# esw0116/DynaVSR

Hardware: AMD Instinct MI355X
Metric: inner-loop frames/sec/GPU (EDVR-M x4, 5x3x180x320): forward leg = BASELINE.json configs[1]; the inner MAML step and the per-frame pipeline are `inner_step` / `per_frame_pipeline` (higher is better)
Workload: dtype f32; 1 GPU; EDVR-M x4 forward (PCD deformable alignment + TSA fusion + reconstruction), clips of 1x5x3x180x320 -> 3x720x1280 (BASELINE.json configs[1]); one step = 2 clip(s) per GPU, one per HIP stream (adapt.super_resolve_video); clips_in_flight_per_gpu=2

## Files before the change

### dynavsr_amd/csrc/conv2d_wino5.hip

```cpp
#include <type_traits>

#include "common.h"
#include "kernels.h"
#include "small_grid.h"

namespace dvsr {

#ifdef DVSR_CONV_TRACE
#define W5_STAMP(i)                                                                                       \
  do {                                                                                                    \
    if (a.trace && threadIdx.x == 0) a.trace[(size_t)blockIdx.x * 64 + (i)] = __builtin_readcyclecounter(); \
  } while (0)
#else
#define W5_STAMP(i) \
  do {              \
  } while (0)
#endif

typedef float w5f2 __attribute__((ext_vector_type(2)));
typedef __bf16 w5bf8 __attribute__((ext_vector_type(8)));
typedef __bf16 w5bf2 __attribute__((ext_vector_type(2)));
typedef unsigned w5u4 __attribute__((ext_vector_type(4)));

constexpr int W5_PCH = 18 * 2 * 3 * 256;

template <int TC>
struct Wino5Shape {
  static constexpr int CC = 8, NTILE = 32, TRW = NTILE / TC, NT = 768;
  static constexpr int OH = 4 * TRW, OW = 4 * TC;
  static constexpr int IH = OH + 2, RP = OW + 8, GR = RP / 4;
  static constexpr int NG = CC * IH * GR;
  static constexpr int NI = (NG + NT - 1) / NT;
  static constexpr int RAWPAD = NI * NT * 4;
  static constexpr int VIMG = 36 * 3 * 32 * 4;
  static constexpr int XCH = 6 * 16 * 64 * 4;
  static constexpr int LOOP = 2 * RAWPAD + 2 * VIMG;
  static constexpr size_t LDS_BYTES = (size_t)(LOOP > XCH ? LOOP : XCH) * sizeof(float);
};

constexpr int w5_waitcnt(int vm, int lgkm) { return (vm & 15) | (7 << 4) | ((lgkm & 15) << 8) | ((vm >> 4) << 14); }

__device__ __forceinline__ unsigned w5_cvt_pk(float a, float b) {
  return __builtin_bit_cast(unsigned, __builtin_convertvector(w5f2{a, b}, w5bf2));
}
__device__ __forceinline__ void w5_dma16(__amdgpu_buffer_rsrc_t rs, float* lds, unsigned voff, unsigned soff) {
  __builtin_amdgcn_raw_ptr_buffer_load_lds(rs, (__attribute__((address_space(3))) void*)lds, 16, voff, soff, 0, 0);
}
__device__ __forceinline__ __amdgpu_buffer_rsrc_t w5_rsrc(const float* base, int num_records) {
  return __builtin_amdgcn_make_buffer_rsrc(const_cast<float*>(base), 0, num_records, 0x00020000);
}

__global__ void pack_weights_wino5_kernel(PackTable t) {
  const PackEntry& e = t.e[blockIdx.y];
  if (e.layout != PackLayout::WINO_F4) return;
  __bf16* const P16 = reinterpret_cast<__bf16*>(e.P);
  const size_t total = (size_t)e.ncb * e.nchunks * 512;
  constexpr double G[6][3] = {{1.0 / 4, 0, 0},          {-1.0 / 6, -1.0 / 6, -1.0 / 6}, {-1.0 / 6, 1.0 / 6, -1.0 / 6},
                              {1.0 / 24, 1.0 / 12, 1.0 / 6}, {1.0 / 24, -1.0 / 12, 1.0 / 6}, {0, 0, 1}};
  for (size_t i = blockIdx.x * (size_t)blockDim.x + threadIdx.x; i < total; i += (size_t)gridDim.x * blockDim.x) {
    const int c8 = (int)(i & 7), col = (int)((i >> 3) & 63);
    const size_t ck = i >> 9;
    const int k = (int)(ck % e.nchunks), cb = (int)(ck / e.nchunks);
    const int co = cb * 64 + col, ci = k * 8 + c8;
    double g[3][3];
    const bool ok = co < e.Cout && ci < e.Ctot;
    const float* src = !e.wt ? e.w + ((size_t)co * (e.w_ctot ? e.w_ctot : e.Ctot) + (e.w_ctot ? e.w_coff : 0) + ci) * 9
                             : e.w + ((size_t)ci * e.w_ctot + e.w_coff + co) * 9;
#pragma unroll
    for (int tap = 0; tap < 9; ++tap) g[tap / 3][tap % 3] = ok ? (double)src[e.wt ? 8 - tap : tap] : 0.0;
    double c[6][3];
#pragma unroll
    for (int xi = 0; xi < 6; ++xi)
#pragma unroll
      for (int b = 0; b < 3; ++b) c[xi][b] = G[xi][0] * g[0][b] + G[xi][1] * g[1][b] + G[xi][2] * g[2][b];
    const int mh = col >> 5, c32 = col & 31;
    __bf16* dst = P16 + ck * (size_t)(2 * W5_PCH) + (size_t)mh * 1536 + (size_t)c32 * 8 + c8;
#pragma unroll
    for (int xi = 0; xi < 6; ++xi)
#pragma unroll
      for (int nu = 0; nu < 6; ++nu) {
        const float u = (float)(c[xi][0] * G[nu][0] + c[xi][1] * G[nu][1] + c[xi][2] * G[nu][2]);
        const __bf16 h = (__bf16)u;
        const float r1 = u - (float)h;
        const __bf16 m = (__bf16)r1;
        const __bf16 l = (__bf16)(r1 - (float)m);
        __bf16* d = dst + (size_t)(xi * 3 + (nu >> 1)) * 3072;
        if (nu & 1) { d[512] = m; d[768] = h; d[1024] = l; }
        else { d[0] = h; d[256] = m; d[1280] = l; }
      }
  }
}

int pack_weights_wino5_run(const PackTable& t, hipStream_t st) {
  hipLaunchKernelGGL(pack_weights_wino5_kernel, dim3(64, t.n), dim3(256), 0, st, t);
  return check_launch("pack_weights_wino5_kernel");
}

template <int TC, bool RES, bool R16, bool PRE>
__global__ __launch_bounds__(1024) void conv2d_wino5_kernel(ConvK2 a) {
  static_assert(!PRE || (R16 && !RES), "the addend is read by the sixteen-reader epilogue, never beside a residual");
  using Sh = Wino5Shape<TC>;
  constexpr int IH = Sh::IH, RP = Sh::RP, GR = Sh::GR;
  constexpr int CHF = IH * RP;
  constexpr int QF = 768 * 4;
  extern __shared__ __attribute__((aligned(16))) float smem[];
  float* const raw0 = smem;
  unsigned* const vimg0 = reinterpret_cast<unsigned*>(smem + 2 * Sh::RAWPAD);

  const int id = blockIdx.x;
  const int q_ = id >> 3;
  const int cbi = q_ % a.ncb;
  const int j_ = q_ / a.ncb;
  const int tile = (id & 7) * a.tiles_per_xcd + j_;
  if (j_ >= a.tiles_per_xcd || tile >= a.ntiles) return;
  const int tx_ = tile % a.tiles_x;
  const int t2 = tile / a.tiles_x;
  const int ty_ = t2 % a.tiles_y;
  const int n = t2 / a.tiles_y;
  const int oy0 = ty_ * Sh::OH, ox0 = tx_ * Sh::OW;

  const int tid = threadIdx.x, lane = tid & 63;
  const int wave = __builtin_amdgcn_readfirstlane(tid >> 6);
  const int lo = lane & 31, hi = lane >> 5;
  const size_t HW = (size_t)a.H * a.W;
  auto fence = [&]() __attribute__((always_inline)) { __builtin_amdgcn_sched_barrier(0); };
  auto lds_barrier = [&]() __attribute__((always_inline)) {
    asm volatile("s_waitcnt lgkmcnt(0)" ::: "memory");
    __builtin_amdgcn_s_barrier();
    asm volatile("" ::: "memory");
  };
  W5_STAMP(0);
#ifdef DVSR_CONV_TRACE
  if (a.trace && threadIdx.x == 0) a.trace[(size_t)blockIdx.x * 64 + 60] = __builtin_amdgcn_s_memrealtime();
#endif

  auto read16 = [&](int m) __attribute__((always_inline)) {
    int le = lane;
    asm volatile("" : "+v"(le));
    const int rq_r = wave & 3, cp_r = wave >> 2;
    const float* const xr = smem + (rq_r * 64 + le) * 4 + cp_r;
    const int lo_e = le & 31, hi_e = le >> 5;
    const int trow_e = lo_e / TC, tcol_e = lo_e - trow_e * TC;
    const int oy = oy0 + 4 * trow_e, ox = ox0 + 4 * tcol_e;
    const size_t HWo = (size_t)a.Ho * a.Wo;
    const float slope = a.act == ACT_LRELU ? 0.1f : (a.act == ACT_RELU ? 0.f : 1.f);
    const float* bias = wset_ptr(a.bias, a.b_gs, n, a.wdiv);
    const int co0 = cbi * 64 + m * 32 + 8 * rq_r + 4 * hi_e + cp_r;
    f32x4 pr[4];
    if constexpr (PRE) {
      const bool live = oy < a.Ho && ox < a.Wo && co0 < a.Cout;
      const float* pre = a.pre + (size_t)(n / a.pre_bdiv) * a.pre_bs + (size_t)co0 * HWo + (size_t)oy * a.Wo + ox;
#pragma unroll
      for (int i = 0; i < 4; ++i)
        pr[i] = (live && oy + i < a.Ho) ? *reinterpret_cast<const f32x4*>(pre + (size_t)i * a.Wo) : f32x4{0.f, 0.f, 0.f, 0.f};
    }
    float y[4][4];
#pragma unroll
    for (int j = 0; j < 4; ++j) {
      float z[6];
#pragma unroll
      for (int x = 0; x < 6; ++x) z[x] = xr[(x * 16 + j * 4) * 256];
      const float sa = z[1] + z[2], da = z[1] - z[2];
      const float sb = z[3] + z[4], db = z[3] - z[4];
      y[0][j] = z[0] + sa + sb;
      y[1][j] = __builtin_fmaf(2.f, db, da);
      y[2][j] = __builtin_fmaf(4.f, sb, sa);
      y[3][j] = __builtin_fmaf(8.f, db, da) + z[5];
    }
    const bool px_ok = oy < a.Ho && ox < a.Wo;
    const int nrow = a.Ho - oy < 4 ? a.Ho - oy : 4;
    if (px_ok && co0 < a.Cout) {
      const float b0 = bias ? bias[co0] : 0.f;
      const size_t base = ((size_t)n * a.Cout + co0) * HWo + (size_t)oy * a.Wo + ox;
      f32x4 rr[4];
      if constexpr (RES) {
#pragma unroll
        for (int i = 0; i < 4; ++i)
          rr[i] = i < nrow ? *reinterpret_cast<const f32x4*>(a.res + base + (size_t)i * a.Wo) : f32x4{0.f, 0.f, 0.f, 0.f};
      }
#pragma unroll
      for (int i = 0; i < 4; ++i) {
        if (i >= nrow) break;
        f32x4 v;
#pragma unroll
        for (int j = 0; j < 4; ++j) {
          float v0 = y[i][j] + b0;
          if constexpr (PRE) v0 += pr[i][j];
          v[j] = fmaxf(v0, v0 * slope);
        }
        if constexpr (RES) v += rr[i];
        *reinterpret_cast<f32x4*>(a.y + base + (size_t)i * a.Wo) = v;
      }
    }
  };

  if (wave >= 12) {
    const int pw = wave - 12, ptid = tid - 768;
    const float* x0n = a.x0 + (size_t)n * a.x0_bs;
    const float* x1n = a.c1 ? a.x1 + (size_t)(n / a.x1_bdiv) * a.x1_bs : x0n;
    static_assert(IH * GR * 4 == 720, "a channel quad is 720 groups");
    unsigned hoff[3];
#pragma unroll
    for (int jj = 0; jj < 3; ++jj) {
      const int L = jj * 256 + ptid;
      const int cq = L / (IH * GR), rr = L - cq * (IH * GR);
      const int iy = rr / GR, g = rr - iy * GR;
      const int gy = oy0 - 1 + iy, gx = ox0 - 4 + 4 * g;
      const bool live = L < 4 * IH * GR;
      const bool ok = live && (unsigned)gy < (unsigned)a.H && (unsigned)gx < (unsigned)a.W;
      hoff[jj] = ok ? (unsigned)(((size_t)cq * HW + (size_t)gy * a.W + gx) * 4) : 0x80000000u;
      if (live && !ok) {
#pragma unroll
        for (int bb = 0; bb < 4; ++bb) *reinterpret_cast<f32x4*>(raw0 + (bb >> 1) * Sh::RAWPAD + (bb & 1) * QF + L * 4) = f32x4{0.f, 0.f, 0.f, 0.f};
      }
    }
    const unsigned chunk_bytes = (unsigned)(Sh::CC * HW * 4), quad_bytes = (unsigned)(4 * HW * 4);
    auto issue_raw = [&](int k) __attribute__((always_inline)) {
      const bool live = k < a.nchunks;
      const bool second = k * Sh::CC >= a.c0;
      const unsigned soff = live ? (unsigned)(second ? k - a.c0 / Sh::CC : k) * chunk_bytes : 0u;
      const __amdgpu_buffer_rsrc_t rs = w5_rsrc(second ? x1n : x0n, live ? 0x7fffffff : 0);
      float* dst = raw0 + (k & 1) * Sh::RAWPAD + 256 * pw;
#pragma unroll
      for (int jj = 0; jj < 3; ++jj) {
        w5_dma16(rs, dst + jj * 1024, hoff[jj], soff);
        w5_dma16(rs, dst + QF + jj * 1024, hoff[jj], soff + quad_bytes);
      }
    };
    const int ptile = 8 * pw + (lane & 7), ppair = (lane >> 3) & 3;
    const int trow_t = ptile / TC, tcol_t = ptile - trow_t * TC;
    const int pch = 2 * ppair + hi;
    const float* prd = raw0 + (pch >> 2) * QF + (pch & 3) * CHF + 4 * trow_t * RP + 4 * tcol_t;
    unsigned* vw12 = vimg0 + (hi ? 2 : 1) * 6 * 384 + ptile * 4 + ppair;
    unsigned* vw34 = vimg0 + (hi ? 4 : 3) * 6 * 384 + ptile * 4 + ppair;
    unsigned* vw05 = vimg0 + (hi ? 5 : 0) * 6 * 384 + ptile * 4 + ppair;
    auto ld_row = [&](float (&d)[6], int row) __attribute__((always_inline)) {
      const float* p = prd + row * RP;
      const w5f2 l2 = *reinterpret_cast<const w5f2*>(p + 2);
      const f32x4 m4 = *reinterpret_cast<const f32x4*>(p + 4);
      const w5f2 h2 = *reinterpret_cast<const w5f2*>(p + 8);
      d[0] = l2[1]; d[1] = m4[0]; d[2] = m4[1]; d[3] = m4[2]; d[4] = m4[3]; d[5] = h2[0];
    };
    auto colpass = [&](const float (&r)[6], float (&v)[6]) __attribute__((always_inline)) {
      v[0] = __builtin_fmaf(4.f, r[0], __builtin_fmaf(-5.f, r[2], r[4]));
      v[5] = __builtin_fmaf(4.f, r[1], __builtin_fmaf(-5.f, r[3], r[5]));
      const float e1 = __builtin_fmaf(-4.f, r[2], r[4]), o1 = __builtin_fmaf(-4.f, r[1], r[3]);
      v[1] = e1 + o1; v[2] = e1 - o1;
      const float e2 = r[4] - r[2], o2 = r[3] - r[1];
      v[3] = __builtin_fmaf(2.f, o2, e2); v[4] = __builtin_fmaf(-2.f, o2, e2);
    };
    auto finish_pair = [&](const float (&ra)[6], const float (&rb)[6], unsigned* vw) __attribute__((always_inline)) {
      float va[6], vb[6];
      colpass(ra, va);
      colpass(rb, vb);
#pragma unroll
      for (int v = 0; v < 6; ++v) {
        const auto s0 = __builtin_amdgcn_permlane32_swap(__builtin_bit_cast(unsigned, va[v]), __builtin_bit_cast(unsigned, vb[v]), false, false);
        const unsigned u0 = s0[0], u1 = s0[1];
        const float v0 = __builtin_bit_cast(float, u0), v1 = __builtin_bit_cast(float, u1);
        const unsigned h = w5_cvt_pk(v0, v1);
        const float r0 = v0 - __builtin_bit_cast(float, h << 16), r1 = v1 - __builtin_bit_cast(float, h & 0xffff0000u);
        const unsigned m = w5_cvt_pk(r0, r1);
        const float q0 = r0 - __builtin_bit_cast(float, m << 16), q1 = r1 - __builtin_bit_cast(float, m & 0xffff0000u);
        unsigned* d = vw + v * 384;
#ifdef W5_NOVW
        d[0] = h ^ m ^ w5_cvt_pk(q0, q1);
#else
        d[0] = h; d[128] = m; d[256] = w5_cvt_pk(q0, q1);
#endif
      }
    };
    auto produce = [&]() __attribute__((always_inline)) {
      float d0[6], d1[6], d2[6], d3[6], d4[6], d5[6];
      ld_row(d1, 1); ld_row(d2, 2); ld_row(d3, 3); ld_row(d4, 4);
      ld_row(d0, 0); ld_row(d5, 5);
      float ra[6], rb[6];
#pragma unroll
      for (int j = 0; j < 6; ++j) {
        const float e = __builtin_fmaf(-4.f, d2[j], d4[j]), o = __builtin_fmaf(-4.f, d1[j], d3[j]);
        ra[j] = e + o; rb[j] = e - o;
      }
      finish_pair(ra, rb, vw12);
      fence();
#pragma unroll
      for (int j = 0; j < 6; ++j) {
        const float e = d4[j] - d2[j], o = d3[j] - d1[j];
        ra[j] = __builtin_fmaf(2.f, o, e); rb[j] = __builtin_fmaf(-2.f, o, e);
      }
      finish_pair(ra, rb, vw34);
      fence();
#pragma unroll
      for (int j = 0; j < 6; ++j) {
        ra[j] = __builtin_fmaf(4.f, d0[j], __builtin_fmaf(-5.f, d2[j], d4[j]));
        rb[j] = __builtin_fmaf(4.f, d1[j], __builtin_fmaf(-5.f, d3[j], d5[j]));
      }
      finish_pair(ra, rb, vw05);
    };
    issue_raw(0);
    issue_raw(1);
    __builtin_amdgcn_s_waitcnt(w5_waitcnt(6, 0));
    __builtin_amdgcn_s_barrier();
    asm volatile("" ::: "memory");
    produce();
    __builtin_amdgcn_s_waitcnt(w5_waitcnt(0, 0));
    __builtin_amdgcn_s_barrier();
    asm volatile("" ::: "memory");
    int vstep = Sh::VIMG, rstep = Sh::RAWPAD;
    vw12 += vstep; vw34 += vstep; vw05 += vstep; prd += rstep;
    __builtin_amdgcn_s_setprio(3);
    for (int k = 0; k < a.nchunks; ++k) {

#ifndef W5_NODMA
      issue_raw(k + 2);
#endif
#ifndef W5_NOPROD
      if (k + 1 < a.nchunks) produce();
#endif
      __builtin_amdgcn_s_waitcnt(w5_waitcnt(0, 0));
      __builtin_amdgcn_s_barrier();
      asm volatile("" ::: "memory");
      vw12 -= vstep; vw34 -= vstep; vw05 -= vstep; prd -= rstep;
      vstep = -vstep; rstep = -rstep;
    }
    if constexpr (R16) {
      __builtin_amdgcn_s_setprio(0);
      lds_barrier();
      lds_barrier(); read16(0);
      lds_barrier();
      lds_barrier(); read16(1);
    } else {
      lds_barrier(); lds_barrier(); lds_barrier(); lds_barrier();
    }
    return;
  }
  {
    const int cxi = wave % 6, cmh = wave / 6;
    f32x16 acc[6];
#pragma unroll
    for (int v = 0; v < 6; ++v)
#pragma unroll
      for (int r = 0; r < 16; ++r) acc[v][r] = 0.f;
    const float* wp_cb = wset_ptr(a.wp, a.w_gs, n, a.wdiv) + (size_t)cbi * a.nchunks * W5_PCH;
    const __amdgpu_buffer_rsrc_t wrsrc = w5_rsrc(wp_cb, -1);
    const unsigned avoff = (unsigned)(lane * 16);
    const int asb = (cxi * 3 * 2 + cmh) * 3072;
    f32x4 AF[3];
    auto gldA = [&](auto g_, int k) __attribute__((always_inline)) {
      constexpr int G = decltype(g_)::value;
#ifdef W5_NOA
      if (k > 0 || G > 2) return;
#endif
      const int soff = k * (W5_PCH * 4) + asb + (G / 3) * 6144 + (G % 3) * 1024;
      AF[G % 3] = __builtin_bit_cast(f32x4, __builtin_amdgcn_raw_buffer_load_b128(wrsrc, (int)avoff, soff, 0));
    };
    auto blend = [&](f32x4& x, const f32x4& l, bool keep) __attribute__((always_inline)) {
#pragma unroll
      for (int r = 0; r < 4; ++r) x[r] = keep ? x[r] : l[r];
    };
    const unsigned* vrd = vimg0 + cxi * 6 * 384 + lo * 4;
    const unsigned* vrd_lh = vrd + (hi ? 0 : 256);
    const unsigned* vrd_hl = vrd + (hi ? 256 : 0);
    w5u4 BF[2];
    auto ldB = [&](auto f_) __attribute__((always_inline)) {
      constexpr int F = decltype(f_)::value, NU = F / 3, W = F % 3;
      if constexpr (W == 0) BF[F & 1] = *reinterpret_cast<const w5u4*>(vrd + NU * 384);
      else if constexpr (W == 1) BF[F & 1] = *reinterpret_cast<const w5u4*>(vrd + NU * 384 + 128);
      else if constexpr (NU & 1) BF[F & 1] = *reinterpret_cast<const w5u4*>(vrd_hl + NU * 384);
      else BF[F & 1] = *reinterpret_cast<const w5u4*>(vrd_lh + NU * 384);
    };
    auto mma = [&](f32x16& c, const f32x4& av, const w5u4& bv) __attribute__((always_inline)) {
#ifdef W5_NOMMA
      c[0] += av[0] * __builtin_bit_cast(float, bv[0]);
      return;
#endif
      c = __builtin_amdgcn_mfma_f32_32x32x16_bf16(__builtin_bit_cast(w5bf8, av), __builtin_bit_cast(w5bf8, bv), c, 0, 0, 0);
    };
    static_for<0, 3>([&](auto g_) __attribute__((always_inline)) { gldA(g_, 0); });
    __builtin_amdgcn_s_barrier();
    asm volatile("" ::: "memory");
    __builtin_amdgcn_s_barrier();
    asm volatile("" ::: "memory");
    int vstep = Sh::VIMG;
    for (int k = 0; k < a.nchunks; ++k) {
      ldB(std::integral_constant<int, 0>{}); ldB(std::integral_constant<int, 1>{});
      const int knext = k + 1 < a.nchunks ? k + 1 : k;
      static_for<0, 18>([&](auto f_) __attribute__((always_inline)) {
        constexpr int F = decltype(f_)::value, NU = F / 3, I = F % 3;
        constexpr int XS = NU & 1;
        mma(acc[NU], AF[XS], BF[F & 1]);
#ifdef W5_NOBR
        if constexpr (false)
#else
        if constexpr (F + 2 < 18)
#endif
          ldB(std::integral_constant<int, (F + 2 < 18 ? F + 2 : 0)>{});
        if constexpr (I == 1) {
          blend(AF[XS], AF[2], (NU & 1) ? hi != 0 : hi == 0);
          if constexpr ((NU & 1) && NU < 5) gldA(std::integral_constant<int, 3 * ((NU < 5 ? NU : 1) / 2) + 5>{}, k);
          if constexpr (NU == 5) gldA(std::integral_constant<int, 2>{}, knext);
        }
        if constexpr (I == 2) {
          if constexpr (NU < 4) gldA(std::integral_constant<int, 3 * ((NU < 4 ? NU : 0) / 2) + 3 + (NU & 1)>{}, k);
          else gldA(std::integral_constant<int, (NU & 1)>{}, knext);
        }
        fence();
      });
      lds_barrier();
      if (k < 16) W5_STAMP(3 + k);
      vrd += vstep; vrd_lh += vstep; vrd_hl += vstep;
      vstep = -vstep;
    }
  W5_STAMP(40);

  int lane_e = lane;
  asm volatile("" : "+v"(lane_e));
  f32x16 Z[4];
#pragma unroll
  for (int r = 0; r < 16; ++r) {
    const float sa = acc[1][r] + acc[2][r], da = acc[1][r] - acc[2][r];
    const float sb = acc[3][r] + acc[4][r], db = acc[3][r] - acc[4][r];
    Z[0][r] = acc[0][r] + sa + sb;
    Z[1][r] = __builtin_fmaf(2.f, db, da);
    Z[2][r] = __builtin_fmaf(4.f, sb, sa);
    Z[3][r] = __builtin_fmaf(8.f, db, da) + acc[5][r];
  }
  float* const xw = smem + (cxi * 16 * 64 + lane_e) * 4;
  const int rq_r = wave & 3, cp_r = wave >> 2;
  const float* const xr = smem + (rq_r * 64 + lane_e) * 4 + cp_r * 2;
  const int lo_e = lane_e & 31, hi_e = lane_e >> 5;
  const int trow_e = lo_e / TC, tcol_e = lo_e - trow_e * TC;
  const int oy = oy0 + 4 * trow_e, ox = ox0 + 4 * tcol_e;
  const size_t HWo = (size_t)a.Ho * a.Wo;
  const float slope = a.act == ACT_LRELU ? 0.1f : (a.act == ACT_RELU ? 0.f : 1.f);
  const float* bias = wset_ptr(a.bias, a.b_gs, n, a.wdiv);
  W5_STAMP(50);
  lds_barrier();
  W5_STAMP(51);
#pragma unroll 1
  for (int m = 0; m < 2; ++m) {
    if (cmh == m) {
#pragma unroll
      for (int j = 0; j < 4; ++j)
#pragma unroll
        for (int rq = 0; rq < 4; ++rq)
          *reinterpret_cast<f32x4*>(xw + (j * 4 + rq) * 256) = f32x4{Z[j][4 * rq], Z[j][4 * rq + 1], Z[j][4 * rq + 2], Z[j][4 * rq + 3]};
    }
    W5_STAMP(52 + 4 * m);
    lds_barrier();
    W5_STAMP(53 + 4 * m);
    if constexpr (R16) read16(m);
    else if (wave < 8) {
      const int co0 = cbi * 64 + m * 32 + 8 * rq_r + 4 * hi_e + 2 * cp_r;
      float y[2][4][4];
#pragma unroll
      for (int j = 0; j < 4; ++j) {
        w5f2 z[6];
#pragma unroll
        for (int x = 0; x < 6; ++x) z[x] = *reinterpret_cast<const w5f2*>(xr + (x * 16 + j * 4) * 256);
#pragma unroll
        for (int c = 0; c < 2; ++c) {
          const float sa = z[1][c] + z[2][c], da = z[1][c] - z[2][c];
          const float sb = z[3][c] + z[4][c], db = z[3][c] - z[4][c];
          y[c][0][j] = z[0][c] + sa + sb;
          y[c][1][j] = __builtin_fmaf(2.f, db, da);
          y[c][2][j] = __builtin_fmaf(4.f, sb, sa);
          y[c][3][j] = __builtin_fmaf(8.f, db, da) + z[5][c];
        }
      }
      const bool px_ok = oy < a.Ho && ox < a.Wo;
      const int nrow = a.Ho - oy < 4 ? a.Ho - oy : 4;
      if (px_ok && co0 < a.Cout) {
        const bool two = co0 + 1 < a.Cout;
        const float b0 = bias ? bias[co0] : 0.f, b1 = (bias && two) ? bias[co0 + 1] : 0.f;
#pragma unroll
        for (int i = 0; i < 4; ++i)
#pragma unroll
          for (int j = 0; j < 4; ++j) {
            const float v0 = y[0][i][j] + b0, v1 = y[1][i][j] + b1;
            y[0][i][j] = fmaxf(v0, v0 * slope);
            y[1][i][j] = fmaxf(v1, v1 * slope);
          }
        if (a.ps == 0) {
#pragma unroll
          for (int c = 0; c < 2; ++c) {
            if (c == 1 && !two) break;
            const size_t base = ((size_t)n * a.Cout + co0 + c) * HWo + (size_t)oy * a.Wo + ox;
            if constexpr (RES) {
              f32x4 rr[4];
#pragma unroll
              for (int i = 0; i < 4; ++i)
                rr[i] = i < nrow ? *reinterpret_cast<const f32x4*>(a.res + base + (size_t)i * a.Wo) : f32x4{0.f, 0.f, 0.f, 0.f};
#pragma unroll
              for (int i = 0; i < 4; ++i) {
                if (i >= nrow) break;
                const f32x4 v = f32x4{y[c][i][0], y[c][i][1], y[c][i][2], y[c][i][3]} + rr[i];
                *reinterpret_cast<f32x4*>(a.y + base + (size_t)i * a.Wo) = v;
              }
            } else {
#pragma unroll
              for (int i = 0; i < 4; ++i) {
                if (i >= nrow) break;
                *reinterpret_cast<f32x4*>(a.y + base + (size_t)i * a.Wo) = f32x4{y[c][i][0], y[c][i][1], y[c][i][2], y[c][i][3]};
              }
            }
          }
        } else {
          const int cq = co0 >> 2, dy = (co0 >> 1) & 1;
          float* dst = a.y + (((size_t)n * (a.Cout >> 2) + cq) * (2 * a.Ho) + (2 * oy + dy)) * (size_t)(2 * a.Wo) + 2 * ox;
#pragma unroll
          for (int i = 0; i < 4; ++i) {
            if (i >= nrow) break;
            float* d = dst + (size_t)(2 * i) * (2 * a.Wo);
            *reinterpret_cast<f32x4*>(d) = f32x4{y[0][i][0], y[1][i][0], y[0][i][1], y[1][i][1]};
            *reinterpret_cast<f32x4*>(d + 4) = f32x4{y[0][i][2], y[1][i][2], y[0][i][3], y[1][i][3]};
          }
        }
      }
    }
    W5_STAMP(54 + 4 * m);
    if (m == 0) lds_barrier();
    W5_STAMP(55 + 4 * m);
  }
#ifdef DVSR_CONV_TRACE
  W5_STAMP(41);
  __builtin_amdgcn_s_waitcnt(0);
  W5_STAMP(42);
  if (a.trace && threadIdx.x == 0) {
    a.trace[(size_t)blockIdx.x * 64 + 61] = __builtin_amdgcn_s_memrealtime();
    a.trace[(size_t)blockIdx.x * 64 + 63] = __builtin_amdgcn_s_getreg((4) | (0 << 6) | (31 << 11));
    a.trace[(size_t)blockIdx.x * 64 + 62] = __builtin_amdgcn_s_getreg((20) | (0 << 6) | (31 << 11));
  }
#endif
  }
}

template <int TC>
static int launch_wino5(ConvK2 k, hipStream_t st) {
  using Sh = Wino5Shape<TC>;
  auto kern = k.pre ? conv2d_wino5_kernel<TC, false, true, true>
                    : (k.res ? conv2d_wino5_kernel<TC, true, true, false> : conv2d_wino5_kernel<TC, false, false, false>);
  static PerDeviceOnce attr_once, attr_once_r, attr_once_p;
  set_dyn_lds_once(attr_once, (const void*)conv2d_wino5_kernel<TC, false, false, false>, Sh::LDS_BYTES);
  set_dyn_lds_once(attr_once_r, (const void*)conv2d_wino5_kernel<TC, true, true, false>, Sh::LDS_BYTES);
  set_dyn_lds_once(attr_once_p, (const void*)conv2d_wino5_kernel<TC, false, true, true>, Sh::LDS_BYTES);
  k.tiles_x = ceil_div(k.Wo, Sh::OW); k.tiles_y = ceil_div(k.Ho, Sh::OH); k.ntiles = k.tiles_x * k.tiles_y * k.N;
  k.ncb = ceil_div(k.Cout, 64);
  k.tiles_per_xcd = ceil_div(k.ntiles, 8);
  k.nitems = k.tiles_per_xcd * 8 * k.ncb;
  hipLaunchKernelGGL(kern, dim3(k.nitems), dim3(1024), Sh::LDS_BYTES, st, k);
  return check_launch("conv2d_wino5_kernel");
}

int conv2d_wino5_launch(const ConvK2& k, int th, hipStream_t st) {
  return th == 16 ? launch_wino5<8>(k, st) : launch_wino5<16>(k, st);
}

}
```

Measured before the change: 259.6 frames/s.

## Prefetch Winograd epilogue bias/residual loads early and skip dead output half-blocks

The R16 epilogue of the Winograd conv kernel now issues its bias and residual/pre-add global loads ahead of the LDS barriers and output transform, so their latency overlaps with the transform and barrier waits. Producer waves prefetch both rounds and compute waves prefetch the next round during the current one. Blocks whose second 32-channel half lies beyond Cout now skip that half's MFMA main loop and epilogue round, while keeping barrier counts matched. The early loads raise register pressure, and the changed barrier sequences must stay aligned across wave roles.

```diff
diff --git a/dynavsr_amd/csrc/conv2d_wino5.hip b/dynavsr_amd/csrc/conv2d_wino5.hip
--- a/dynavsr_amd/csrc/conv2d_wino5.hip
+++ b/dynavsr_amd/csrc/conv2d_wino5.hip
@@ -21,6 +21,12 @@
 typedef __bf16 w5bf8 __attribute__((ext_vector_type(8)));
 typedef __bf16 w5bf2 __attribute__((ext_vector_type(2)));
 typedef unsigned w5u4 __attribute__((ext_vector_type(4)));
+
+#ifdef W5_LATE_LOADS
+constexpr bool W5_EARLY = false;
+#else
+constexpr bool W5_EARLY = true;
+#endif
 
 constexpr int W5_PCH = 18 * 2 * 3 * 256;
 
@@ -123,6 +129,8 @@
   const int wave = __builtin_amdgcn_readfirstlane(tid >> 6);
   const int lo = lane & 31, hi = lane >> 5;
   const size_t HW = (size_t)a.H * a.W;
+  const bool dead1 = cbi * 64 + 32 >= a.Cout;
+  const int nround = dead1 ? 1 : 2;
   auto fence = [&]() __attribute__((always_inline)) { __builtin_amdgcn_sched_barrier(0); };
   auto lds_barrier = [&]() __attribute__((always_inline)) {
     asm volatile("s_waitcnt lgkmcnt(0)" ::: "memory");
@@ -134,9 +142,26 @@
   if (a.trace && threadIdx.x == 0) a.trace[(size_t)blockIdx.x * 64 + 60] = __builtin_amdgcn_s_memrealtime();
 #endif
 
-  auto read16 = [&](int m) __attribute__((always_inline)) {
-    int le = lane;
-    asm volatile("" : "+v"(le));
+  struct Ep16 { float b0; f32x4 row[4]; };
+  auto fetch16 = [&](int m, int le, Ep16& e) __attribute__((always_inline)) {
+    const int rq_r = wave & 3, cp_r = wave >> 2;
+    const int lo_e = le & 31, hi_e = le >> 5;
+    const int trow_e = lo_e / TC, tcol_e = lo_e - trow_e * TC;
+    const int oy = oy0 + 4 * trow_e, ox = ox0 + 4 * tcol_e;
+    const size_t HWo = (size_t)a.Ho * a.Wo;
+    const float* bias = wset_ptr(a.bias, a.b_gs, n, a.wdiv);
+    const int co0 = cbi * 64 + m * 32 + 8 * rq_r + 4 * hi_e + cp_r;
+    const bool live = oy < a.Ho && ox < a.Wo && co0 < a.Cout;
+    e.b0 = (bias && live) ? bias[co0] : 0.f;
+    if constexpr (RES || PRE) {
+      const float* src = RES ? a.res + ((size_t)n * a.Cout + co0) * HWo + (size_t)oy * a.Wo + ox
+                             : a.pre + (size_t)(n / a.pre_bdiv) * a.pre_bs + (size_t)co0 * HWo + (size_t)oy * a.Wo + ox;
+#pragma unroll
+      for (int i = 0; i < 4; ++i)
+        e.row[i] = (live && oy + i < a.Ho) ? *reinterpret_cast<const f32x4*>(src + (size_t)i * a.Wo) : f32x4{0.f, 0.f, 0.f, 0.f};
+    }
+  };
+  auto read16 = [&](int m, int le, Ep16& e) __attribute__((always_inline)) {
     const int rq_r = wave & 3, cp_r = wave >> 2;
     const float* const xr = smem + (rq_r * 64 + le) * 4 + cp_r;
     const int lo_e = le & 31, hi_e = le >> 5;
@@ -146,13 +171,12 @@
     const float slope = a.act == ACT_LRELU ? 0.1f : (a.act == ACT_RELU ? 0.f : 1.f);
     const float* bias = wset_ptr(a.bias, a.b_gs, n, a.wdiv);
     const int co0 = cbi * 64 + m * 32 + 8 * rq_r + 4 * hi_e + cp_r;
-    f32x4 pr[4];
-    if constexpr (PRE) {
+    if constexpr (PRE && !W5_EARLY) {
       const bool live = oy < a.Ho && ox < a.Wo && co0 < a.Cout;
       const float* pre = a.pre + (size_t)(n / a.pre_bdiv) * a.pre_bs + (size_t)co0 * HWo + (size_t)oy * a.Wo + ox;
 #pragma unroll
       for (int i = 0; i < 4; ++i)
-        pr[i] = (live && oy + i < a.Ho) ? *reinterpret_cast<const f32x4*>(pre + (size_t)i * a.Wo) : f32x4{0.f, 0.f, 0.f, 0.f};
+        e.row[i] = (live && oy + i < a.Ho) ? *reinterpret_cast<const f32x4*>(pre + (size_t)i * a.Wo) : f32x4{0.f, 0.f, 0.f, 0.f};
     }
     float y[4][4];
 #pragma unroll
@@ -167,17 +191,31 @@
       y[2][j] = __builtin_fmaf(4.f, sb, sa);
       y[3][j] = __builtin_fmaf(8.f, db, da) + z[5];
     }
+#ifdef DVSR_CONV_TRACE
+    asm volatile("s_waitcnt lgkmcnt(0)" ::: "memory");
+    W5_STAMP(43 + 2 * m);
+    if constexpr (W5_EARLY) asm volatile("s_waitcnt vmcnt(0)" ::: "memory");
+    if constexpr (W5_EARLY) W5_STAMP(44 + 2 * m);
+#endif
     const bool px_ok = oy < a.Ho && ox < a.Wo;
     const int nrow = a.Ho - oy < 4 ? a.Ho - oy : 4;
     if (px_ok && co0 < a.Cout) {
-      const float b0 = bias ? bias[co0] : 0.f;
       const size_t base = ((size_t)n * a.Cout + co0) * HWo + (size_t)oy * a.Wo + ox;
-      f32x4 rr[4];
-      if constexpr (RES) {
-#pragma unroll
-        for (int i = 0; i < 4; ++i)
-          rr[i] = i < nrow ? *reinterpret_cast<const f32x4*>(a.res + base + (size_t)i * a.Wo) : f32x4{0.f, 0.f, 0.f, 0.f};
-      }
+      if constexpr (!W5_EARLY) {
+        e.b0 = bias ? bias[co0] : 0.f;
+        if constexpr (RES) {
+#pragma unroll
+          for (int i = 0; i < 4; ++i)
+            e.row[i] = i < nrow ? *reinterpret_cast<const f32x4*>(a.res + base + (size_t)i * a.Wo) : f32x4{0.f, 0.f, 0.f, 0.f};
+        }
+      }
+#ifdef DVSR_CONV_TRACE
+      if constexpr (!W5_EARLY) {
+        asm volatile("s_waitcnt vmcnt(0)" ::: "memory");
+        W5_STAMP(44 + 2 * m);
+      }
+#endif
+      const float b0 = e.b0;
 #pragma unroll
       for (int i = 0; i < 4; ++i) {
         if (i >= nrow) break;
@@ -185,10 +223,10 @@
 #pragma unroll
         for (int j = 0; j < 4; ++j) {
           float v0 = y[i][j] + b0;
-          if constexpr (PRE) v0 += pr[i][j];
+          if constexpr (PRE) v0 += e.row[i][j];
           v[j] = fmaxf(v0, v0 * slope);
         }
-        if constexpr (RES) v += rr[i];
+        if constexpr (RES) v += e.row[i];
         *reinterpret_cast<f32x4*>(a.y + base + (size_t)i * a.Wo) = v;
       }
     }
@@ -324,12 +362,22 @@
     }
     if constexpr (R16) {
       __builtin_amdgcn_s_setprio(0);
+      int le = lane;
+      asm volatile("" : "+v"(le));
+      Ep16 e0, e1;
+      if constexpr (W5_EARLY) {
+        fetch16(0, le, e0);
+        if (nround == 2) fetch16(1, le, e1);
+      }
       lds_barrier();
-      lds_barrier(); read16(0);
-      lds_barrier();
-      lds_barrier(); read16(1);
+      lds_barrier(); read16(0, le, e0);
+      if (nround == 2) {
+        lds_barrier();
+        lds_barrier(); read16(1, le, e1);
+      }
     } else {
-      lds_barrier(); lds_barrier(); lds_barrier(); lds_barrier();
+      lds_barrier(); lds_barrier();
+      if (nround == 2) { lds_barrier(); lds_barrier(); }
     }
     return;
   }
@@ -375,40 +423,48 @@
 #endif
       c = __builtin_amdgcn_mfma_f32_32x32x16_bf16(__builtin_bit_cast(w5bf8, av), __builtin_bit_cast(w5bf8, bv), c, 0, 0, 0);
     };
-    static_for<0, 3>([&](auto g_) __attribute__((always_inline)) { gldA(g_, 0); });
-    __builtin_amdgcn_s_barrier();
-    asm volatile("" ::: "memory");
-    __builtin_amdgcn_s_barrier();
-    asm volatile("" ::: "memory");
-    int vstep = Sh::VIMG;
-    for (int k = 0; k < a.nchunks; ++k) {
-      ldB(std::integral_constant<int, 0>{}); ldB(std::integral_constant<int, 1>{});
-      const int knext = k + 1 < a.nchunks ? k + 1 : k;
-      static_for<0, 18>([&](auto f_) __attribute__((always_inline)) {
-        constexpr int F = decltype(f_)::value, NU = F / 3, I = F % 3;
-        constexpr int XS = NU & 1;
-        mma(acc[NU], AF[XS], BF[F & 1]);
+    if (dead1 && cmh == 1) {
+      __builtin_amdgcn_s_barrier();
+      asm volatile("" ::: "memory");
+      __builtin_amdgcn_s_barrier();
+      asm volatile("" ::: "memory");
+      for (int k = 0; k < a.nchunks; ++k) lds_barrier();
+    } else {
+      static_for<0, 3>([&](auto g_) __attribute__((always_inline)) { gldA(g_, 0); });
+      __builtin_amdgcn_s_barrier();
+      asm volatile("" ::: "memory");
+      __builtin_amdgcn_s_barrier();
+      asm volatile("" ::: "memory");
+      int vstep = Sh::VIMG;
+      for (int k = 0; k < a.nchunks; ++k) {
+        ldB(std::integral_constant<int, 0>{}); ldB(std::integral_constant<int, 1>{});
+        const int knext = k + 1 < a.nchunks ? k + 1 : k;
+        static_for<0, 18>([&](auto f_) __attribute__((always_inline)) {
+          constexpr int F = decltype(f_)::value, NU = F / 3, I = F % 3;
+          constexpr int XS = NU & 1;
+          mma(acc[NU], AF[XS], BF[F & 1]);
 #ifdef W5_NOBR
-        if constexpr (false)
+          if constexpr (false)
 #else
-        if constexpr (F + 2 < 18)
-#endif
-          ldB(std::integral_constant<int, (F + 2 < 18 ? F + 2 : 0)>{});
-        if constexpr (I == 1) {
-          blend(AF[XS], AF[2], (NU & 1) ? hi != 0 : hi == 0);
-          if constexpr ((NU & 1) && NU < 5) gldA(std::integral_constant<int, 3 * ((NU < 5 ? NU : 1) / 2) + 5>{}, k);
-          if constexpr (NU == 5) gldA(std::integral_constant<int, 2>{}, knext);
-        }
-        if constexpr (I == 2) {
-          if constexpr (NU < 4) gldA(std::integral_constant<int, 3 * ((NU < 4 ? NU : 0) / 2) + 3 + (NU & 1)>{}, k);
-          else gldA(std::integral_constant<int, (NU & 1)>{}, knext);
-        }
-        fence();
-      });
-      lds_barrier();
-      if (k < 16) W5_STAMP(3 + k);
-      vrd += vstep; vrd_lh += vstep; vrd_hl += vstep;
-      vstep = -vstep;
+          if constexpr (F + 2 < 18)
+#endif
+            ldB(std::integral_constant<int, (F + 2 < 18 ? F + 2 : 0)>{});
+          if constexpr (I == 1) {
+            blend(AF[XS], AF[2], (NU & 1) ? hi != 0 : hi == 0);
+            if constexpr ((NU & 1) && NU < 5) gldA(std::integral_constant<int, 3 * ((NU < 5 ? NU : 1) / 2) + 5>{}, k);
+            if constexpr (NU == 5) gldA(std::integral_constant<int, 2>{}, knext);
+          }
+          if constexpr (I == 2) {
+            if constexpr (NU < 4) gldA(std::integral_constant<int, 3 * ((NU < 4 ? NU : 0) / 2) + 3 + (NU & 1)>{}, k);
+            else gldA(std::integral_constant<int, (NU & 1)>{}, knext);
+          }
+          fence();
+        });
+        lds_barrier();
+        if (k < 16) W5_STAMP(3 + k);
+        vrd += vstep; vrd_lh += vstep; vrd_hl += vstep;
+        vstep = -vstep;
+      }
     }
   W5_STAMP(40);
 
@@ -423,6 +479,12 @@
     Z[1][r] = __builtin_fmaf(2.f, db, da);
     Z[2][r] = __builtin_fmaf(4.f, sb, sa);
     Z[3][r] = __builtin_fmaf(8.f, db, da) + acc[5][r];
+  }
+  Ep16 ep;
+  if constexpr (R16 && W5_EARLY) {
+    int le0 = lane_e;
+    asm volatile("" : "+v"(le0) : "v"(Z[0]), "v"(Z[1]), "v"(Z[2]), "v"(Z[3]));
+    fetch16(0, le0, ep);
   }
   float* const xw = smem + (cxi * 16 * 64 + lane_e) * 4;
   const int rq_r = wave & 3, cp_r = wave >> 2;
@@ -437,7 +499,7 @@
   lds_barrier();
   W5_STAMP(51);
 #pragma unroll 1
-  for (int m = 0; m < 2; ++m) {
+  for (int m = 0; m < nround; ++m) {
     if (cmh == m) {
 #pragma unroll
       for (int j = 0; j < 4; ++j)
@@ -448,8 +510,16 @@
     W5_STAMP(52 + 4 * m);
     lds_barrier();
     W5_STAMP(53 + 4 * m);
-    if constexpr (R16) read16(m);
-    else if (wave < 8) {
+    if constexpr (R16) {
+      read16(m, lane_e, ep);
+      if constexpr (W5_EARLY) {
+        if (m + 1 < nround) {
+          int le1 = lane_e;
+          asm volatile("" : "+v"(le1));
+          fetch16(m + 1, le1, ep);
+        }
+      }
+    } else if (wave < 8) {
       const int co0 = cbi * 64 + m * 32 + 8 * rq_r + 4 * hi_e + 2 * cp_r;
       float y[2][4][4];
 #pragma unroll
@@ -467,11 +537,19 @@
           y[c][3][j] = __builtin_fmaf(8.f, db, da) + z[5][c];
         }
       }
+#ifdef DVSR_CONV_TRACE
+      asm volatile("s_waitcnt lgkmcnt(0)" ::: "memory");
+      W5_STAMP(43 + 2 * m);
+#endif
       const bool px_ok = oy < a.Ho && ox < a.Wo;
       const int nrow = a.Ho - oy < 4 ? a.Ho - oy : 4;
       if (px_ok && co0 < a.Cout) {
         const bool two = co0 + 1 < a.Cout;
         const float b0 = bias ? bias[co0] : 0.f, b1 = (bias && two) ? bias[co0 + 1] : 0.f;
+#ifdef DVSR_CONV_TRACE
+        asm volatile("s_waitcnt vmcnt(0)" ::: "memory");
+        W5_STAMP(44 + 2 * m);
+#endif
 #pragma unroll
         for (int i = 0; i < 4; ++i)
 #pragma unroll
@@ -518,7 +596,7 @@
       }
     }
     W5_STAMP(54 + 4 * m);
-    if (m == 0) lds_barrier();
+    if (m + 1 < nround) lds_barrier();
     W5_STAMP(55 + 4 * m);
   }
 #ifdef DVSR_CONV_TRACE
```

Result: no change. 261.5 frames/s (median of 6 runs) (+0.7%).
